# delldu/VSTNet

Measured on AMD Instinct MI355X. Metric: stylized frames/sec at 1024x1024 (1/2/4/8 GPU) + % HBM roofline, higher is better.
Workload: dtype bf16x3

## Files before the change

### include/vstnet.h

```cpp
#ifndef VSTNET_H
#define VSTNET_H

#include <stddef.h>
#include <stdint.h>

#ifdef __cplusplus
extern "C" {
#endif
#pragma GCC visibility push(default)

#define VST_OK 0
#define VST_E_ARG (-1)
#define VST_E_SHAPE (-2)
#define VST_E_MODE (-3)
#define VST_E_WORKSPACE (-4)

#define VST_PREC_BF16X3 0
#define VST_PREC_FP32 1
#define VST_PREC_F16X2 2

#define VST_PREC_F16X2H 3

#define VST_NUM_BLOCKS 32

// ... 128 lines not shown
int vst_cwct_factor_n(const double* content_stats, const double* const* style_stats_host_array, const float* alphas_host,
                      int n_styles, float alpha_c, float eps, int N, float* affine, int* info, void* workspace,
                      size_t workspace_bytes, void* stream);
int vst_cwct_prefactor_n(const double* stats, int N, float eps, double* out, int* info, void* workspace, size_t workspace_bytes,
                         void* stream);
int vst_cwct_apply_n(const float* x, float* y, int N, long L, const float* affine, const uint8_t* mask, int label, void* stream);
size_t vst_cwct_stats_n_f64_workspace_bytes(int N, long L);
int vst_cwct_stats_n_f64(const float* x, int N, long L, const uint8_t* mask, int label, double* stats, void* workspace,
                         size_t workspace_bytes, void* stream);
size_t vst_cwct_factor_n_f64_workspace_bytes(int N);
int vst_cwct_factor_n_f64(const double* content_stats, const double* const* style_stats_host_array, const float* alphas_host,
                          int n_styles, float alpha_c, float eps, int N, double* affine, int* info, void* workspace,
                          size_t workspace_bytes, void* stream);
int vst_cwct_apply_n_f64(const float* x, float* y, int N, long L, const double* affine, const uint8_t* mask, int label,
                         void* stream);

#define VST_KERNEL_ID(cin, cout, stride) (((cin) << 16) | ((cout) << 4) | (stride))
#define VST_KERNEL_ALL (-1)
#define VST_KERNEL_PACK 1
#define VST_KERNEL_UNPACK 2
#define VST_KERNEL_SPREAD 3
#define VST_KERNEL_GATHER 4
#define VST_KERNEL_CWCT_STATS 5
#define VST_KERNEL_CWCT_FACTOR 6
#define VST_KERNEL_CWCT_APPLY 7
#define VST_KERNEL_PRESPLIT 8
int vst_profile_begin(int kernel_id, int max_records);
int vst_profile_end(double* total_ms, int* launches);
int vst_profile_end_table(int* ids, double* ms, int* launches, int cap, int* n_ids);

#define VST_OPT_STAGE3_LEAN 1
#define VST_OPT_STAGE3_PINGPONG 2
#define VST_OPT_STAGE3_WIDE 3
int vst_set_option(int option, int value);
int vst_get_option(int option);

#pragma GCC visibility pop
#ifdef __cplusplus
}
#endif
#endif
```

### vstnet_amd/_lib.py

```python
from __future__ import annotations

import ctypes as C
import glob
import os
import subprocess

PKG_DIR = os.path.dirname(os.path.abspath(__file__))
REPO_DIR = os.path.dirname(PKG_DIR)
LIB_PATH = os.environ.get("VSTNET_HIP_LIB") or os.path.join(PKG_DIR, "libvstnet_hip.so")
RESOURCES_PATH = os.path.join(PKG_DIR, "libvstnet_hip.resources.txt")
SOURCES = sorted(glob.glob(os.path.join(PKG_DIR, "csrc", "*.hip")))
HEADERS = sorted(glob.glob(os.path.join(PKG_DIR, "csrc", "*.h"))) + [os.path.join(REPO_DIR, "include", "vstnet.h")]

NUM_BLOCKS = 32
PREC_BF16X3 = 0
PREC_FP32 = 1
PREC_F16X2 = 2
PREC_F16X2H = 3

EXPORTS = [
    "vst_version", "vst_error_string", "vst_conv_packed_bytes", "vst_pack_conv", "vst_pack_input",
    "vst_unpack_output", "vst_pack_input_u8", "vst_unpack_output_u8", "vst_revnet_forward_u8", "vst_revnet_inverse_u8",
    "vst_spread", "vst_gather", "vst_block_tmp_bytes", "vst_block_apply",
    "vst_pass_workspace_bytes", "vst_revnet_forward", "vst_revnet_inverse",
    "vst_cwct_stats_workspace_bytes", "vst_cwct_stats", "vst_cwct_factor", "vst_cwct_apply", "vst_cwct_apply_prec",
    "vst_cwct_prefactor", "vst_label_plan", "vst_cwct_labels_workspace_bytes", "vst_cwct_stats_labels",
    "vst_cwct_factor_labels", "vst_cwct_apply_labels", "vst_profile_begin", "vst_profile_end", "vst_profile_end_table", "vst_lab_luminance",
    "vst_revnet_encode", "vst_revnet_encode_u8", "vst_revnet_decode", "vst_revnet_decode_u8", "vst_code_to_z", "vst_z_to_code",
    "vst_cwct_stats_code_workspace_bytes", "vst_cwct_stats_code", "vst_cwct_apply_code",
    "vst_mask_to_code", "vst_cwct_stats_labels_code_workspace_bytes", "vst_cwct_stats_labels_code", "vst_cwct_apply_labels_code",
    "vst_revnet_decode_labels", "vst_revnet_decode_labels_u8", "vst_pass_sub_batch",
    "vst_normalize_block", "vst_range_flags", "vst_range_flags_async",
    "vst_cwct_stats_f64_workspace_bytes", "vst_cwct_stats_f64", "vst_cwct_factor_f64_workspace_bytes", "vst_cwct_factor_f64",
    "vst_cwct_apply_f64",
    "vst_generic_conv", "vst_generic_squeeze", "vst_generic_unsqueeze", "vst_generic_copy_channels", "vst_generic_zero",
    "vst_set_option", "vst_get_option",
    "vst_cwct_stats_n_workspace_bytes", "vst_cwct_stats_n", "vst_cwct_factor_n_workspace_bytes", "vst_cwct_factor_n",
    "vst_cwct_prefactor_n", "vst_cwct_apply_n", "vst_cwct_stats_n_f64_workspace_bytes", "vst_cwct_stats_n_f64",
    "vst_cwct_factor_n_f64_workspace_bytes", "vst_cwct_factor_n_f64", "vst_cwct_apply_n_f64",
    "vst_max_frame_pixels", "vst_cwct_stats_code_rect", "vst_cwct_stats_labels_code_rect",
]
OPT_STAGE3_LEAN = 1
OPT_STAGE3_PINGPONG = 2
OPT_STAGE3_WIDE = 3
RANGE_SATURATED = 1
RANGE_WEIGHT = 2


PRECISIONS = {"bf16x3": PREC_BF16X3, "fp32": PREC_FP32, "f16x2": PREC_F16X2, "f16x2h": PREC_F16X2H}


def default_precision() -> str:
    p = os.environ.get("VST_PRECISION", "bf16x3")
    if p not in PRECISIONS:
        raise ValueError(f"VST_PRECISION must be one of {sorted(PRECISIONS)}")
    return p


class VstError(RuntimeError):
    pass


class ConvWeights(C.Structure):
    _fields_ = [("packed", C.c_void_p), ("bias", C.c_void_p)]


class BlockWeights(C.Structure):
    _fields_ = [("conv", ConvWeights * 3)]


class NetWeights(C.Structure):
    _fields_ = [("blocks", BlockWeights * NUM_BLOCKS)]


def build(force: bool = False, verbose: bool = False) -> str:
    newest_src = max(os.path.getmtime(p) for p in SOURCES + HEADERS)
    if not force and os.path.exists(LIB_PATH) and os.path.getmtime(LIB_PATH) >= newest_src:
# ... 185 lines not shown
```

### vstnet_amd/csrc/conv.hip

```cpp
#include <mutex>
#include <stdlib.h>
#include "common.h"

#ifndef VST_ABLATE
#define VST_ABLATE 0
#endif

struct ConvArgs {
    const float* in;
    float* out;
    const unsigned char* packed;
    const float* bias;
    int Hin, Win, Hout, Wout;
    int Wq;
    size_t in_img_stride;
    size_t out_img_stride;
    float sign;
    int tiles_x, tiles_y, tiles_total;
    const unsigned char* packed1;
    const float* bias1;
    unsigned char* out_sp;
    size_t out_sp_img_bytes;
    unsigned trace_base;
};
// ... 721 lines not shown
        vst_pp_clk[2 * (i_)] = __builtin_amdgcn_s_memtime();                                                     \
        vst_pp_clk[2 * (i_) + 1] = __builtin_amdgcn_s_memrealtime();                                             \
    }
#else
#define PP_STAMP(grp_, st_, k_)
#define PP_CLK(i_)
#endif
template <int CIN, int COUT, int NW_ = 8, int MR_ = 2>
struct PipeCfg {
    static constexpr int NW = NW_, NTHR = 64 * NW, MR = MR_;
    static constexpr int NT = 64, NB = 4, TH = MR * NW, IW = 18, NPIX = (TH + 2) * IW, NSLOT = (NPIX + 15) / 16 * 16;
    static constexpr int NCHUNK = CIN / 32, NCOT = COUT / 64;
    static constexpr int A_PLANE = 4 * NSLOT * 16, A_BUF = 2 * A_PLANE;
    static constexpr int B_PLANE = 3 * 4 * 64 * 16, B_BUF = 2 * B_PLANE;
    static constexpr int LDS_BYTES = 2 * A_BUF + 2 * B_BUF;
    static constexpr int A_PART = NPIX * 4 / 3;
    static constexpr int A_ITEMS = ((A_PART / 4 + 15) / 16 * 64 + NTHR - 1) / NTHR;
    static constexpr int B_ITEMS = 2 * 768 / NTHR;
    static_assert(NPIX % 3 == 0, "three equal parts");
    static_assert(LDS_BYTES <= 160 * 1024, "LDS budget");
};

template <int NDSR, int NVM, int NDW>
__device__ __forceinline__ void wide_interleave() {
#pragma unroll
    for (int i = 0; i < 48; ++i) {
        __builtin_amdgcn_sched_group_barrier(0x008, 1, 0);
        if (i % 2 == 0 && i / 2 < NDSR) __builtin_amdgcn_sched_group_barrier(0x100, 1, 0);
        if (i % 2 == 1 && i / 2 < NVM) __builtin_amdgcn_sched_group_barrier(0x020, 1, 0);
        if (i % 2 == 1 && i / 2 < NDW) __builtin_amdgcn_sched_group_barrier(0x200, 1, 0);
    }
}

template <int CIN, int COUT, bool IN_STATE, bool OUT_STATE, int NW = 8, int MR = 2>
__global__ __launch_bounds__(64 * NW, (NW == 4 && MR == 2) ? 2 : 1) void conv_pipe_kernel(const ConvArgs a) {
    using C = PipeCfg<CIN, COUT, NW, MR>;
    constexpr bool WIDE = NW == 4 && MR == 4;
    extern __shared__ __attribute__((aligned(16))) unsigned char smem[];
    unsigned char* const Abuf = smem;
    unsigned char* const Bbuf = smem + 2 * C::A_BUF;

    const int tid = threadIdx.x, lane = tid & 63, wave = tid >> 6;
    const int lrow = lane & 15, kg = lane >> 4;
    int bx, by, b;
    if (!xcd_tile(a, bx, by, b)) return;
    VST_TRACE_BEGIN(4)
    PP_CLK(0)
    const int tx0 = bx * 16, ty0 = by * C::TH;
    const float* const in_img = a.in + (size_t)b * a.in_img_stride;
    float* const out_img = a.out + (size_t)b * a.out_img_stride;
    const PackedConvLayout PL = packed_conv_layout(COUT, CIN);
    const unsigned char* const w_plane0 = a.packed + PL.f32_bytes;

    unsigned a_src[3][C::A_ITEMS], a_dst[3][C::A_ITEMS];
#pragma unroll
    for (int part = 0; part < 3; ++part)
#pragma unroll
        for (int it = 0; it < C::A_ITEMS; ++it) {
            const int j = it * C::NTHR + tid;
            int sl = (j >> 6) * 16 + (j & 15);
            sl = sl < C::A_PART / 4 ? sl : C::A_PART / 4 - 1;
            const int cig = (j >> 4) & 3, slot = part * (C::A_PART / 4) + sl;
            const int iy = slot / C::IW, ix = slot - iy * C::IW;
            const int gy = reflect_clamp(ty0 - 1 + iy, a.Hin), gx = reflect_clamp(tx0 - 1 + ix, a.Win);
            const size_t off = IN_STATE ? zc_offset(vst_level_of_channels(CIN), gy, gx, a.Wq)
                                        : ((size_t)gy * a.Win + gx) * CIN;
            a_src[part][it] = (unsigned)(off + cig * 8);
            a_dst[part][it] = (cig * C::NSLOT + slot) * 16;
        }
    typedef f32x4 APart[C::A_ITEMS][2];
    typedef u32x4 BStage[C::B_ITEMS];
#define LOAD_A(r, chunk, part)                                                          \
    _Pragma("unroll") for (int it_ = 0; it_ < C::A_ITEMS; ++it_) {                      \
// ... 22 lines not shown
            const int k3 = r >> 8, kgi = (r >> 6) & 3, co = r & 63;
            b_off[it] = (int)(plane * PL.frag_bytes) + ((k3 * 4 + kgi) * COUT + co) * 16;
            b_dst[it] = plane * C::B_PLANE + r * 16;
        }
    }
#define LOAD_B(r, q_, dy_)                                                              \
    {                                                                                   \
        const int cot_ = (q_) / C::NCHUNK, chunk_ = (q_) - cot_ * C::NCHUNK;            \
        const unsigned char* src_ = w_plane0 + ((size_t)(chunk_ * 9 + (dy_) * 3) * 4 * COUT + cot_ * 64) * 16;   \
        _Pragma("unroll") for (int it_ = 0; it_ < C::B_ITEMS; ++it_) r[it_] = *(const u32x4*)(src_ + b_off[it_]); \
    }
#define STORE_B(buf, r)                                                                 \
    { _Pragma("unroll") for (int it_ = 0; it_ < C::B_ITEMS; ++it_) *(u32x4*)(Bbuf + (buf) * C::B_BUF + b_dst[it_]) = r[it_]; }
    struct Frags { bf16x8 wh[4], wl[4], xh[C::MR], xl[C::MR]; };
    auto read_frags = [&](Frags& f, const unsigned char* Ab, const unsigned char* Bb, int k3) {
#pragma unroll
        for (int n = 0; n < 4; ++n) {
            f.wh[n] = __builtin_bit_cast(bf16x8, *(const uint4*)(Bb + (k3 * 256 + n * 16) * 16));
            f.wl[n] = __builtin_bit_cast(bf16x8, *(const uint4*)(Bb + C::B_PLANE + (k3 * 256 + n * 16) * 16));
        }
#pragma unroll
        for (int m = 0; m < C::MR; ++m) {
            f.xh[m] = __builtin_bit_cast(bf16x8, *(const uint4*)(Ab + (m * C::IW + k3) * 16));
            f.xl[m] = __builtin_bit_cast(bf16x8, *(const uint4*)(Ab + C::A_PLANE + (m * C::IW + k3) * 16));
        }
    };

    constexpr int Q = C::NCOT * C::NCHUNK;
    static_assert(Q % 2 == 0, "stage parity is static only for an even number of (slice, chunk) pairs");
    constexpr bool ONE_SET = NW == 4 && !WIDE;
#define RS(i_) (ONE_SET ? 0 : (i_))
    BStage rb[ONE_SET ? 1 : 2];
    APart ra[ONE_SET ? 1 : 2];
    {
        BStage rb0;
        LOAD_B(rb0, 0, 0);
        APart r0, r1, r2;
        LOAD_A(r0, 0, 0); LOAD_A(r1, 0, 1); LOAD_A(r2, 0, 2);
        LOAD_B(rb[RS(1)], 0, 1);
        if (C::NCHUNK > 1) LOAD_A(ra[RS(1)], 1, 0);
        STORE_A(0, 0, r0); STORE_A(0, 1, r1); STORE_A(0, 2, r2);
        STORE_B(0, rb0);
    }
    __syncthreads();

    f32x4 acc[C::MR][4];
#pragma unroll
    for (int m = 0; m < C::MR; ++m)
#pragma unroll
        for (int n = 0; n < 4; ++n) acc[m][n] = f32x4{0.f, 0.f, 0.f, 0.f};
    const int slot_base = (wave * C::MR) * C::IW + lrow;
    const int oy0 = ty0 + wave * C::MR;
    float4 bias[4], old[C::MR][4];
#if VST_ABLATE & 8
    f32x16 abl_big[2];
#pragma unroll
    for (int i = 0; i < 16; ++i) { abl_big[0][i] = 0.f; abl_big[1][i] = 0.f; }
#endif
    const bool full_tile = ty0 + C::TH <= a.Hout && tx0 + 16 <= a.Wout;
    constexpr bool DEFER = OUT_STATE && C::NCOT > 1 && C::NCHUNK == 2 && !VST_PIPE_NO_DEFER;
    bool pending = false;
    int pend_cot = 0;
#define DEFER_UNIT(unit_)                                                                                                             \
    {                                                                                                                                 \
        const int m_ = (unit_) >> 2, n_ = (unit_) & 3;                                                                                \
        if (pending) {                                                             \
            float4* p_ = full_tile ? out_ptr<COUT, OUT_STATE, true>(a, out_img, oy0 + m_, tx0 + lrow, pend_cot * 64 + 4 * kg + n_ * 16) \
                                   : out_ptr<COUT, OUT_STATE, false>(a, out_img, oy0 + m_, tx0 + lrow, pend_cot * 64 + 4 * kg + n_ * 16); \
            if (full_tile || p_) *p_ = old[m_][n_];                                                                                   \
        }                                                                                                                             \
        if (VST_PIPE_OLD_SPREAD) {                                             \
            const float4* q_ = full_tile ? out_ptr<COUT, OUT_STATE, true>(a, out_img, oy0 + m_, tx0 + lrow, cot * 64 + 4 * kg + n_ * 16) \
                                         : out_ptr<COUT, OUT_STATE, false>(a, out_img, oy0 + m_, tx0 + lrow, cot * 64 + 4 * kg + n_ * 16); \
            old[m_][n_] = (full_tile || q_) ? *q_ : make_float4(0.f, 0.f, 0.f, 0.f);                                                  \
        }                                                                                                                             \
    }

#pragma unroll 1
    for (int q0 = 0; q0 < Q; q0 += 2) {
#pragma unroll
      for (int qq = 0; qq < 2; ++qq) {
        const int q = q0 + qq;
        const int cot = q / C::NCHUNK, chunk = q - cot * C::NCHUNK;
        const bool last_chunk = chunk == C::NCHUNK - 1;
#pragma unroll
        for (int dy = 0; dy < 3; ++dy) {
            const int s = q * 3 + dy;
            const int cur = (qq * 3 + dy) & 1;
            if constexpr (WIDE) {
                constexpr bool A_ALWAYS = C::NCOT == 1;
                const int q2 = dy == 0 ? q : q + 1, dy2 = (dy + 2) % 3;
                const int qn = dy == 2 ? q + 1 : q, dyn = (dy + 1) % 3;
                if (DEFER ? (dy == 2 && last_chunk) : (dy == 0 && chunk == 0)) load_bias<COUT, 4>(a, cot * 64 + 4 * kg, bias);
                if (!A_ALWAYS && q < C::NCHUNK - 1) STORE_A((chunk + 1) & 1, dy, ra[cur ^ 1]);
                if (!A_ALWAYS && qn < C::NCHUNK - 1) LOAD_A(ra[cur], qn + 1, dyn);
                if (OUT_STATE && !(DEFER && VST_PIPE_OLD_SPREAD) && dy == 2 && last_chunk) {
                    if (full_tile) load_old<COUT, C::MR, 4, true>(a, out_img, oy0, tx0 + lrow, cot * 64 + 4 * kg, old);
                    else load_old<COUT, C::MR, 4, false>(a, out_img, oy0, tx0 + lrow, cot * 64 + 4 * kg, old);
                }
                const unsigned char* Ab = Abuf + (chunk & 1) * C::A_BUF + (kg * C::NSLOT + slot_base + dy * C::IW) * 16;
                const unsigned char* Bb = Bbuf + (s & 1) * C::B_BUF + (kg * 64 + lrow) * 16;
                Frags fr[2];
#pragma unroll
                for (int k3 = 0; k3 < 3; ++k3) {
                    if constexpr (DEFER) {
                        if (qq == 0 && dy * 3 + k3 < C::MR * 2) { DEFER_UNIT(2 * (dy * 3 + k3)); DEFER_UNIT(2 * (dy * 3 + k3) + 1); }
                    }
                    if (k3 == 0) read_frags(fr[0], Ab, Bb, 0);
                    __builtin_amdgcn_sched_barrier(0);
                    if (k3 == 0) {
                        LOAD_B(rb[cur], q2 < Q ? q2 : Q - 1, dy2);
                        if (A_ALWAYS) LOAD_A(ra[cur], qn + 1 < C::NCHUNK ? qn + 1 : C::NCHUNK - 1, dyn);
                    }
                    if (k3 < 2) read_frags(fr[(k3 + 1) & 1], Ab, Bb, k3 + 1);
                    if (k3 == 2) {
                        STORE_B((s + 1) & 1, rb[cur ^ 1]);
                        if (A_ALWAYS) STORE_A((chunk + 1) & 1, dy, ra[cur ^ 1]);
                    }
                    const Frags& f = fr[k3 & 1];
#pragma unroll
                    for (int m = 0; m < C::MR; ++m)
#pragma unroll
                        for (int n = 0; n < 4; ++n) { MFMA3(acc[m][n], f.wh[n], f.wl[n], f.xh[m], f.xl[m]); }
                    constexpr int NSTG = A_ALWAYS ? C::B_ITEMS + 2 * C::A_ITEMS : C::B_ITEMS;
                    if (k3 == 0) wide_interleave<16, NSTG, 0>();
                    else if (k3 == 1) wide_interleave<16, 0, 0>();
                    else wide_interleave<0, 0, NSTG>();
                    __builtin_amdgcn_sched_barrier(0);
// ... 67 lines not shown
            } else
            if (dy == 2 && last_chunk && (!(VST_ABLATE & 4) || cot == C::NCOT - 1)) {
                if (full_tile) store_tile<COUT, OUT_STATE, C::MR, 4, true>(a, out_img, oy0, tx0 + lrow, cot * 64 + 4 * kg, acc, bias, old);
                else store_tile<COUT, OUT_STATE, C::MR, 4, false>(a, out_img, oy0, tx0 + lrow, cot * 64 + 4 * kg, acc, bias, old);
#pragma unroll
                for (int m = 0; m < C::MR; ++m)
#pragma unroll
                    for (int n = 0; n < 4; ++n) acc[m][n] = f32x4{0.f, 0.f, 0.f, 0.f};
            }
            if (DEFER && qq == 0 && dy == 2) pending = false;
            if ((VST_ABLATE & 4) && dy == 2 && last_chunk && cot != C::NCOT - 1) {
#pragma unroll
                for (int m = 0; m < C::MR; ++m)
#pragma unroll
                    for (int n = 0; n < 4; ++n) asm volatile("" : "+v"(acc[m][n]));
            }
            if (!(VST_ABLATE & 16)) __syncthreads();
        }
      }
    }
#undef LOAD_A
#undef STORE_A
#undef LOAD_B
#undef STORE_B
#undef F4_
#undef RS
#undef DEFER_UNIT
#if VST_ABLATE & 8
    asm volatile("" :: "v"(abl_big[0]), "v"(abl_big[1]));
#endif
    PP_CLK(1)
    VST_TRACE_END_(4, CIN, COUT)
}

#ifndef VST_WITH_PINGPONG
#define VST_WITH_PINGPONG 0
#endif
#if VST_WITH_PINGPONG
template <int CIN, int COUT, bool IN_STATE, bool OUT_STATE>
__global__ __launch_bounds__(512) void conv_pp_kernel(const ConvArgs a) {
    using C = PipeCfg<CIN, COUT, 8>;
    constexpr int SY = 256;
    constexpr int A_ITEMS_Y = ((C::A_PART / 4 + 15) / 16 * 64 + SY - 1) / SY;
    constexpr int B_ITEMS_Y = 2 * 768 / SY;
    extern __shared__ __attribute__((aligned(16))) unsigned char smem[];
    unsigned char* const Abuf = smem;
    unsigned char* const Bbuf = smem + 2 * C::A_BUF;
    float* const bias_lds = (float*)(smem + C::LDS_BYTES);

    const int tid = threadIdx.x, lane = tid & 63, wave = __builtin_amdgcn_readfirstlane(tid >> 6);
    const int lrow = lane & 15, kg = lane >> 4;
    const bool grpY = wave >= 4;
    int bx, by, b;
    if (!xcd_tile(a, bx, by, b)) return;
    VST_TRACE_BEGIN(4)
    PP_CLK(0)
    const int tx0 = bx * 16, ty0 = by * C::TH;
    const float* const in_img = a.in + (size_t)b * a.in_img_stride;
    float* const out_img = a.out + (size_t)b * a.out_img_stride;
    const PackedConvLayout PL = packed_conv_layout(COUT, CIN);
    const unsigned char* const w_plane0 = a.packed + PL.f32_bytes;
    constexpr int Q = C::NCOT * C::NCHUNK, S = 3 * Q;
    constexpr bool A_IN_LOOP = C::NCHUNK > 2;

#define PP_A_ADDR(j_, part_, src_, dst_)                                                                         \
    {                                                                                                            \
// ... 298 lines not shown
static int g_prof_id[VST_PROFILE_MAX_RECORDS];
static hipEvent_t g_prof_ev[2 * VST_PROFILE_MAX_RECORDS];
static bool g_prof_ev_created = false;

int vst_prof_open(int kernel_id, hipStream_t st) {
    const int sel = g_prof_kernel.load(std::memory_order_relaxed);
    if (sel != kernel_id && sel != VST_KERNEL_ALL) return -1;
    std::lock_guard<std::mutex> lk(g_prof_mu);
    if ((g_prof_kernel.load() != kernel_id && g_prof_kernel.load() != VST_KERNEL_ALL) || g_prof_count >= g_prof_cap) return -1;
    const int rec = g_prof_count++;
    g_prof_id[rec] = kernel_id;
    (void)hipEventRecord(g_prof_ev[2 * rec], st);
    return rec;
}

void vst_prof_close(int rec, hipStream_t st) {
    std::lock_guard<std::mutex> lk(g_prof_mu);
    if (rec < g_prof_count) (void)hipEventRecord(g_prof_ev[2 * rec + 1], st);
}

#ifndef VST_LEAN_DEFAULT
#define VST_LEAN_DEFAULT 0
#endif
static std::atomic<int> g_opt_lean{[] { const char* e = getenv("VST_LEAN"); return e && (e[0] == '0' || e[0] == '1') ? e[0] - '0' : VST_LEAN_DEFAULT; }()};
static bool vst_lean_stage3() { return g_opt_lean.load(std::memory_order_relaxed) != 0; }
#ifndef VST_WIDE_DEFAULT
#define VST_WIDE_DEFAULT 1
#endif
static std::atomic<int> g_opt_wide{[] { const char* e = getenv("VST_WIDE"); return e && (e[0] == '0' || e[0] == '1') ? e[0] - '0' : VST_WIDE_DEFAULT; }()};
#ifndef VST_PINGPONG_DEFAULT
#define VST_PINGPONG_DEFAULT 0
#endif
static std::atomic<int> g_opt_pp{[] { const char* e = getenv("VST_PINGPONG"); return e && (e[0] == '0' || e[0] == '1') ? e[0] - '0' : VST_PINGPONG_DEFAULT; }()};

template <int CIN, int COUT, int STRIDE, bool IN_STATE, bool OUT_STATE>
static int launch_conv(const ConvArgs& a, int B, int precision, hipStream_t st, bool out_h16 = false) {
    if (precision == VST_PREC_FP32) {
        const size_t total = (size_t)B * a.Hout * a.Wout * COUT;
        size_t blocks = (total + 255) / 256;
        if (blocks > 65536) blocks = 65536;
        conv_fp32_kernel<IN_STATE, OUT_STATE><<<dim3((unsigned)blocks), 256, 0, st>>>(a, CIN, COUT, STRIDE, B);
        VST_RETURN_IF_LAUNCH_FAILED();
        return VST_OK;
    }
    if (precision != VST_PREC_BF16X3 && !vst_is_f16(precision)) return VST_E_MODE;
    vst_prof_scope prof(VST_KERNEL_ID(CIN, COUT, STRIDE), st);
    if constexpr (CIN >= 64 && COUT >= 64 && STRIDE == 1) {
        ConvArgs t = a;
        t.tiles_x = (a.Wout + 15) / 16;
        if (vst_lean_stage3()) {
            using C = PipeCfg<CIN, COUT, 4>;
            auto kern = conv_pipe_kernel<CIN, COUT, IN_STATE, OUT_STATE, 4>;
            static std::atomic<unsigned> attr_done{0};
            if (int rc_ = vst_ensure_dynamic_lds((const void*)kern, (int)(C::LDS_BYTES), &attr_done)) return rc_;
            t.tiles_y = (a.Hout + C::TH - 1) / C::TH; t.tiles_total = t.tiles_x * t.tiles_y * B;
            VST_TRACE_RESERVE(t, (t.tiles_total + 7) / 8 * 8)
            kern<<<dim3((t.tiles_total + 7) / 8 * 8), C::NTHR, C::LDS_BYTES, st>>>(t);
        } else if (g_opt_wide.load(std::memory_order_relaxed)) {
            using C = PipeCfg<CIN, COUT, 4, 4>;
            auto kern = conv_pipe_kernel<CIN, COUT, IN_STATE, OUT_STATE, 4, 4>;
            static std::atomic<unsigned> attr_done{0};
            if (int rc_ = vst_ensure_dynamic_lds((const void*)kern, (int)(C::LDS_BYTES), &attr_done)) return rc_;
            t.tiles_y = (a.Hout + C::TH - 1) / C::TH; t.tiles_total = t.tiles_x * t.tiles_y * B;
            VST_TRACE_RESERVE(t, (t.tiles_total + 7) / 8 * 8)
            kern<<<dim3((t.tiles_total + 7) / 8 * 8), C::NTHR, C::LDS_BYTES, st>>>(t);
#if VST_WITH_PINGPONG
// ... 65 lines not shown
template <int MID, int CH>
static int launch_pair(const ConvArgs& a, int B, int precision, hipStream_t st) {
    constexpr int T2 = 2;
    const bool t2 = T2 == 2 && vst_is_f16(precision);
    if (precision == VST_PREC_F16X2H) {
        using P = PairCfg<MID, CH, 2, 4, true>;
        vst_prof_scope prof(VST_KERNEL_ID(MID, CH, 1), st);
        auto kern = conv_pair_kernel<MID, CH, 2, 4, true>;
        static std::atomic<unsigned> attr_h16{0};
        if (int rc_ = vst_ensure_dynamic_lds((const void*)kern, P::LDS_BYTES, &attr_h16)) return rc_;
        ConvArgs t = a;
        t.tiles_x = (a.Wout + 15) / 16; t.tiles_y = (a.Hout + 15) / 16; t.tiles_total = t.tiles_x * t.tiles_y * B;
        VST_TRACE_RESERVE(t, (t.tiles_total + 7) / 8 * 8)
        kern<<<dim3((t.tiles_total + 7) / 8 * 8), 256, P::LDS_BYTES, st>>>(t);
        VST_RETURN_IF_LAUNCH_FAILED();
        return VST_OK;
    }
    vst_prof_scope prof(VST_KERNEL_ID(MID, CH, 1), st);
    constexpr int MRT = (MID == 16 && VST_PAIR_MR2) ? 2 : 4;
    constexpr int MRT3 = (MID == 16 && VST_PAIR_MR2_T3) ? 2 : 4;
    auto kern = t2 ? conv_pair_kernel<MID, CH, T2, MRT> : conv_pair_kernel<MID, CH, 3, MRT3>;
    const int lds = t2 ? PairCfg<MID, CH, T2, MRT>::LDS_BYTES : PairCfg<MID, CH, 3, MRT3>::LDS_BYTES;
    const int th = t2 ? 4 * MRT : 4 * MRT3;
    static std::atomic<unsigned> attr_done[2];
    if (int rc_ = vst_ensure_dynamic_lds((const void*)kern, lds, &attr_done[t2 ? 1 : 0])) return rc_;
    ConvArgs t = a;
    t.tiles_x = (a.Wout + 15) / 16; t.tiles_y = (a.Hout + th - 1) / th; t.tiles_total = t.tiles_x * t.tiles_y * B;
    VST_TRACE_RESERVE(t, (t.tiles_total + 7) / 8 * 8)
    kern<<<dim3((t.tiles_total + 7) / 8 * 8), 256, lds, st>>>(t);
    VST_RETURN_IF_LAUNCH_FAILED();
    return VST_OK;
}

template <int CH, int STRIDE>
static int run_block(const vst_block_weights* w, int direction, int precision, float* dst, const float* src,
                     float* tmp, int B, int H, int W, hipStream_t st) {
    constexpr int LV = CH == 16 ? 0 : (CH == 64 ? 1 : 2);
    constexpr int MID = CH / 4;
    constexpr int IN_CH = STRIDE == 1 ? CH : CH / 4;
    const int Ho = H >> LV, Wo = W >> LV;
    const size_t state_img = (size_t)H * W * 16;
    const size_t mid_img = (size_t)Ho * Wo * MID;
    float* h1 = tmp;
    float* h2 = tmp + (size_t)B * mid_img;
    ConvArgs a{};
    a.Wq = W >> 2;
    a.in = src; a.out = h1; a.packed = (const unsigned char*)w->conv[0].packed; a.bias = w->conv[0].bias;
    a.Hin = Ho * STRIDE; a.Win = Wo * STRIDE; a.Hout = Ho; a.Wout = Wo;
    a.in_img_stride = state_img; a.out_img_stride = mid_img; a.sign = 0.f;
    if constexpr (CH == 256 && STRIDE == 2) {
        if (vst_is_f16(precision)) {
            const size_t mid_bytes = (size_t)Ho * Wo * 64 * 4, state_bytes = (size_t)Ho * Wo * 256 * 4;
            unsigned char* const h1p = (unsigned char*)tmp;
            unsigned char* const h2p = h1p + (size_t)B * mid_bytes;
            unsigned char* const planes_a = h2p + (size_t)B * mid_bytes;
            (void)state_bytes;
            a.out_sp = h1p; a.out_sp_img_bytes = mid_bytes;
            int rc2 = launch_conv_s2_planes(a, B, st);
            if (rc2) return rc2;
            const int h2_single = precision == VST_PREC_F16X2H;
            rc2 = vst3_conv_mid(&w->conv[1], h1p, h2p, h2_single, B, H, W, st);
            if (rc2) return rc2;
            return vst3_conv_out(&w->conv[2], h2p, h2_single, dst, direction > 0 ? planes_a : nullptr, direction > 0 ? 1.f : -1.f,
                                 B, H, W, st);
        }
    }
    const bool h16 = CH <= 64 && VST_PAIR && precision == VST_PREC_F16X2H;
    int rc = launch_conv<IN_CH, MID, STRIDE, true, false>(a, B, precision, st, h16);
    if (rc) return rc;
    if constexpr (CH <= 64 && VST_PAIR) {
        if (precision != VST_PREC_FP32) {
            a.in = h1; a.out = dst; a.Hin = Ho; a.Win = Wo; a.in_img_stride = mid_img; a.out_img_stride = state_img;
            a.packed = (const unsigned char*)w->conv[2].packed; a.bias = w->conv[2].bias;
            a.packed1 = (const unsigned char*)w->conv[1].packed; a.bias1 = w->conv[1].bias;
            a.sign = direction > 0 ? 1.f : -1.f;
            return launch_pair<MID, CH>(a, B, precision, st);
        }
    }
    a.in = h1; a.out = h2; a.packed = (const unsigned char*)w->conv[1].packed; a.bias = w->conv[1].bias;
    a.Hin = Ho; a.Win = Wo; a.in_img_stride = mid_img;
    rc = launch_conv<MID, MID, 1, false, false>(a, B, precision, st);
    if (rc) return rc;
    a.in = h2; a.out = dst; a.packed = (const unsigned char*)w->conv[2].packed; a.bias = w->conv[2].bias;
    a.out_img_stride = state_img; a.sign = direction > 0 ? 1.f : -1.f;
    return launch_conv<MID, CH, 1, false, true>(a, B, precision, st);
}

static const int kBlockChannel[VST_NUM_BLOCKS] = {16, 16, 16, 16, 16, 16, 16, 16, 16, 16, 64, 64, 64, 64, 64, 64,
                                                  64, 64, 64, 64, 256, 256, 256, 256, 256, 256, 256, 256, 256, 256,
                                                  256, 256};
static const int kBlockStride[VST_NUM_BLOCKS] = {1, 1, 1, 1, 1, 1, 1, 1, 1, 1, 2, 1, 1, 1, 1, 1,
                                                 1, 1, 1, 1, 2, 1, 1, 1, 1, 1, 1, 1, 1, 1, 1, 1};

VST_DEFINE_TU_RANGE(vst_range_tu_conv)

extern "C" {

int vst_set_option(int option, int value) {
    if (option == VST_OPT_STAGE3_LEAN) g_opt_lean.store(value != 0, std::memory_order_relaxed);
    else if (option == VST_OPT_STAGE3_WIDE) g_opt_wide.store(value != 0, std::memory_order_relaxed);
    else if (option == VST_OPT_STAGE3_PINGPONG && VST_WITH_PINGPONG) g_opt_pp.store(value != 0, std::memory_order_relaxed);
    else return VST_E_ARG;
    return VST_OK;
}

int vst_get_option(int option) {
    if (option == VST_OPT_STAGE3_LEAN) return g_opt_lean.load(std::memory_order_relaxed);
    if (option == VST_OPT_STAGE3_WIDE) return g_opt_wide.load(std::memory_order_relaxed);
    if (option == VST_OPT_STAGE3_PINGPONG && VST_WITH_PINGPONG) return g_opt_pp.load(std::memory_order_relaxed);
    return VST_E_ARG;
}

int vst_range_flags(unsigned* flags_host, int reset) {
    if (!flags_host) return VST_E_ARG;
    hipError_t e = hipDeviceSynchronize();
    if (e != hipSuccess) return (int)e;
    unsigned v = 0;
    if (int rc = vst_range_tu_conv(&v, reset)) return rc;
    if (int rc = vst_range_tu_conv3(&v, reset)) return rc;
    if (int rc = vst_range_tu_layout(&v, reset)) return rc;
    if (int rc = vst_range_tu_cwct(&v, reset)) return rc;
    *flags_host = v;
    return VST_OK;
}

int vst_range_flags_async(unsigned* flags4_dev, void* stream) {
    if (!flags4_dev) return VST_E_ARG;
    hipStream_t st = (hipStream_t)stream;
    if (int rc = vst_range_tu_conv_async(flags4_dev + 0, st)) return rc;
    if (int rc = vst_range_tu_conv3_async(flags4_dev + 1, st)) return rc;
    if (int rc = vst_range_tu_layout_async(flags4_dev + 2, st)) return rc;
    return vst_range_tu_cwct_async(flags4_dev + 3, st);
}

int vst_profile_begin(int kernel_id, int max_records) {
    if ((kernel_id <= 0 && kernel_id != VST_KERNEL_ALL) || max_records <= 0) return VST_E_ARG;
    if (max_records > VST_PROFILE_MAX_RECORDS) max_records = VST_PROFILE_MAX_RECORDS;
    std::lock_guard<std::mutex> lk(g_prof_mu);
    if (!g_prof_ev_created) {
        for (int i = 0; i < 2 * VST_PROFILE_MAX_RECORDS; ++i) {
            hipError_t e = hipEventCreate(&g_prof_ev[i]);
            if (e != hipSuccess) return (int)e;
// ... 335 lines not shown
```

### vstnet_amd/csrc/layout.hip

```cpp
#include "common.h"

__global__ __launch_bounds__(256) void pack_input_kernel(const float* __restrict__ x, float* __restrict__ s1,
                                                         int C, int H, int W, const float* __restrict__ addk) {
    const int xg = blockIdx.x * 64 + (threadIdx.x & 63);
    const int yg = blockIdx.y * 4 + (threadIdx.x >> 6);
    const int b = blockIdx.z;
    if (xg >= W || yg >= H) return;
    const size_t plane = (size_t)H * W;
    const float* src = x + (size_t)b * C * plane + (size_t)yg * W + xg;
    float v[16];
#pragma unroll
    for (int c = 0; c < 16; ++c) v[c] = (c < C ? src[c * plane] : 0.f) + (addk ? addk[c] : 0.f);
    float* dst = s1 + (size_t)b * plane * 16 + zc_offset(0, yg, xg, W >> 2);
#pragma unroll
    for (int c = 0; c < 16; c += 4) *(float4*)(dst + c) = make_float4(v[c], v[c + 1], v[c + 2], v[c + 3]);
}

__global__ __launch_bounds__(256) void unpack_output_kernel(const float* __restrict__ s1, float* __restrict__ x,
                                                            int C, int H, int W) {
    const int xg = blockIdx.x * 64 + (threadIdx.x & 63);
    const int yg = blockIdx.y * 4 + (threadIdx.x >> 6);
    const int b = blockIdx.z;
    if (xg >= W || yg >= H) return;
    const size_t plane = (size_t)H * W;
// ... 199 lines not shown
}

__global__ __launch_bounds__(256) void normalize_block_kernel(float* __restrict__ w1, float* __restrict__ b1, float* __restrict__ w4,
                                                              float* __restrict__ b4, float* __restrict__ w7, int cin1, int mid,
                                                              int cout, float* __restrict__ scales) {
    __shared__ float sc[64];
    const int tid = threadIdx.x, lane = tid & 63, wave = tid >> 6;
    auto row_scales = [&](const float* w, int K) {
        for (int r = wave; r < mid; r += 4) {
            float acc = 0.f;
            for (int k = lane; k < K; k += 64) { const float v = w[(size_t)r * K + k]; acc += v * v; }
#pragma unroll
            for (int o = 32; o >= 1; o >>= 1) acc += __shfl_xor(acc, o, 64);
            if (lane == 0) sc[r] = pow2_scale_of_norm(acc);
        }
        __syncthreads();
    };
    const int K1 = cin1 * 9, K4 = mid * 9;
    row_scales(w1, K1);
    for (int i = tid; i < mid * K1; i += 256) w1[i] *= sc[i / K1];
    for (int i = tid; i < mid; i += 256) { b1[i] *= sc[i]; if (scales) scales[i] = sc[i]; }
    for (int i = tid; i < mid * K4; i += 256) w4[i] /= sc[(i / 9) % mid];
    __syncthreads();
    row_scales(w4, K4);
    for (int i = tid; i < mid * K4; i += 256) w4[i] *= sc[i / K4];
    for (int i = tid; i < mid; i += 256) { b4[i] *= sc[i]; if (scales) scales[mid + i] = sc[i]; }
    for (int i = tid; i < cout * K4; i += 256) w7[i] /= sc[(i / 9) % mid];
}

VST_DEFINE_TU_RANGE(vst_range_tu_layout)

extern "C" {

int vst_version(void) { return 104; }
int64_t vst_max_frame_pixels(void) { return VST_MAX_FRAME_PIXELS; }

int vst_normalize_block(float* w1, float* b1, float* w4, float* b4, float* w7, int c_in1, int c_mid, int c_out, float* scales,
                        void* stream) {
    if (!w1 || !b1 || !w4 || !b4 || !w7) return VST_E_ARG;
    if (c_in1 <= 0 || c_mid <= 0 || c_mid > 64 || c_out <= 0) return VST_E_SHAPE;
    normalize_block_kernel<<<dim3(1), 256, 0, (hipStream_t)stream>>>(w1, b1, w4, b4, w7, c_in1, c_mid, c_out, scales);
    VST_RETURN_IF_LAUNCH_FAILED();
    return VST_OK;
}

const char* vst_error_string(int code) {
    switch (code) {
        case VST_OK: return "ok";
        case VST_E_ARG: return "invalid argument (null pointer or non-positive size)";
        case VST_E_SHAPE: return "unsupported shape (H, W must be multiples of 4 and >= 8, H * W <= VST_MAX_FRAME_PIXELS; channels in the documented sets)";
        case VST_E_MODE: return "unknown mode (precision / sp_steps / direction)";
        case VST_E_WORKSPACE: return "workspace too small or null";
        default: return code > 0 ? hipGetErrorString((hipError_t)code) : "unknown vstnet error";
    }
}

size_t vst_conv_packed_bytes(int cout, int cin) {
    const PackedConvLayout L = packed_conv_layout(cout, cin);
    return L.f16_offset + L.frag_bytes;
}

int vst_pack_conv(const float* w, int cout, int cin, void* packed, void* stream) {
    if (!w || !packed || cout <= 0) return VST_E_ARG;
    if (!(cin == 4 || cin == 16 || (cin >= 32 && cin % 32 == 0))) return VST_E_SHAPE;
    const PackedConvLayout L = packed_conv_layout(cout, cin);
    size_t n = (size_t)9 * cin * cout;
    const size_t n_frag = (size_t)L.ksteps * 4 * L.coutp * 8;
// ... 98 lines not shown
```

Measured before the change: 221.2.

## Fuse conv.4 into conv.7 for 256-channel stage-3 blocks via LDS halo tile

For 256-channel blocks in bf16x3 with the wide path, the middle 64->64 conv is now computed inside the 64->256 conv kernel. Each tile loads a 20x20 halo of h1 into LDS, computes the 18x18 h2 region (interior plus ring) with MFMA, applies bias, ReLU and reflect padding, and writes h2 into LDS where the next conv reads it. This removes the h2 round-trip through HBM and one launch, at the cost of recomputing halo pixels, higher LDS use and register pressure. It is on by default and can be turned off through an option or environment variable.

```diff
diff --git a/include/vstnet.h b/include/vstnet.h
--- a/include/vstnet.h
+++ b/include/vstnet.h
@@ -184,6 +184,7 @@
 #define VST_OPT_STAGE3_LEAN 1
 #define VST_OPT_STAGE3_PINGPONG 2
 #define VST_OPT_STAGE3_WIDE 3
+#define VST_OPT_STAGE3_PAIR 4
 int vst_set_option(int option, int value);
 int vst_get_option(int option);
 
diff --git a/vstnet_amd/_lib.py b/vstnet_amd/_lib.py
--- a/vstnet_amd/_lib.py
+++ b/vstnet_amd/_lib.py
@@ -43,6 +43,7 @@
 OPT_STAGE3_LEAN = 1
 OPT_STAGE3_PINGPONG = 2
 OPT_STAGE3_WIDE = 3
+OPT_STAGE3_PAIR = 4
 RANGE_SATURATED = 1
 RANGE_WEIGHT = 2
 
diff --git a/vstnet_amd/csrc/conv.hip b/vstnet_amd/csrc/conv.hip
--- a/vstnet_amd/csrc/conv.hip
+++ b/vstnet_amd/csrc/conv.hip
@@ -777,13 +777,67 @@
     }
 }
 
-template <int CIN, int COUT, bool IN_STATE, bool OUT_STATE, int NW = 8, int MR = 2>
+struct S3PairCfg {
+    static constexpr int R1 = 20, N1SLOT = R1 * R1;
+    static constexpr int A1_PLANE = 4 * N1SLOT * 16, A1_BUF = 2 * A1_PLANE;
+    static constexpr int H1_ITEMS = (4 * N1SLOT + 255) / 256;
+    static constexpr int NRING = 2 * 18 + 2 * 16;
+    static constexpr int B_OFF = 2 * A1_BUF;
+    static constexpr int LDS_BYTES = B_OFF + 2 * PipeCfg<64, 256, 4, 4>::B_BUF;
+    static_assert(2 * PipeCfg<64, 256, 4, 4>::A_BUF <= B_OFF, "the h2 images fit over the h1 images");
+    static_assert(LDS_BYTES <= 160 * 1024, "LDS budget");
+};
+
+__device__ __forceinline__ void s3_ring_pos(int p, int& ry, int& rx) {
+    if (p < 36) {
+        ry = p < 18 ? 0 : 17;
+        rx = p < 18 ? p : p - 18;
+    } else {
+        ry = (p < 52 ? p - 36 : p - 52) + 1;
+        rx = p < 52 ? 0 : 17;
+    }
+}
+
+__device__ __forceinline__ void s3_put_h2(unsigned char* smem, const f32x4& acc, const float4& bias, int n, int kg, int ry, int rx,
+                                          bool ok, bool ring_in, int ty0, int tx0, int H, int W) {
+    using C7 = PipeCfg<64, 256, 4, 4>;
+    float4 r = make_float4(acc[0] + bias.x, acc[1] + bias.y, acc[2] + bias.z, acc[3] + bias.w);
+    r.x = r.x > 0.f ? r.x : 0.f; r.y = r.y > 0.f ? r.y : 0.f;
+    r.z = r.z > 0.f ? r.z : 0.f; r.w = r.w > 0.f ? r.w : 0.f;
+    uint2 h, l;
+    split4(r, h, l);
+    unsigned char* const base = smem + (n >> 1) * C7::A_BUF + ((n & 1) * 2 + (kg >> 1)) * C7::NSLOT * 16 + (kg & 1) * 8;
+#define S3_PUT(slot_)                                                                              \
+    {                                                                                              \
+        *(uint2*)(base + (slot_) * 16) = h;                                                        \
+        *(uint2*)(base + C7::A_PLANE + (slot_) * 16) = l;                                          \
+    }
+    if (ring_in) {
+        if (ok) S3_PUT(ry * C7::IW + rx);
+    } else {
+        const int gy = ty0 - 1 + ry, gx = tx0 - 1 + rx;
+        if (ok && gy >= 0 && gy < H && gx >= 0 && gx < W) {
+            const int my = gy == 1 ? -2 : (gy == H - 2 ? 2 : 0), mx = gx == 1 ? -2 : (gx == W - 2 ? 2 : 0);
+            int sy = ry + my, sx = rx + mx;
+            sy = (sy < 0 || sy >= 18) ? ry : sy;
+            sx = (sx < 0 || sx >= 18) ? rx : sx;
+            S3_PUT(ry * C7::IW + rx);
+            S3_PUT(sy * C7::IW + rx);
+            S3_PUT(ry * C7::IW + sx);
+            S3_PUT(sy * C7::IW + sx);
+        }
+    }
+#undef S3_PUT
+}
+
+template <int CIN, int COUT, bool IN_STATE, bool OUT_STATE, int NW = 8, int MR = 2, bool S3PAIR = false>
 __global__ __launch_bounds__(64 * NW, (NW == 4 && MR == 2) ? 2 : 1) void conv_pipe_kernel(const ConvArgs a) {
     using C = PipeCfg<CIN, COUT, NW, MR>;
     constexpr bool WIDE = NW == 4 && MR == 4;
+    static_assert(!S3PAIR || (WIDE && CIN == 64 && COUT == 256 && !IN_STATE && OUT_STATE), "the fused form: conv.7 of the 256-channel blocks");
     extern __shared__ __attribute__((aligned(16))) unsigned char smem[];
     unsigned char* const Abuf = smem;
-    unsigned char* const Bbuf = smem + 2 * C::A_BUF;
+    unsigned char* const Bbuf = smem + (S3PAIR ? S3PairCfg::B_OFF : 2 * C::A_BUF);
 
     const int tid = threadIdx.x, lane = tid & 63, wave = tid >> 6;
     const int lrow = lane & 15, kg = lane >> 4;
@@ -872,7 +926,128 @@
 #define RS(i_) (ONE_SET ? 0 : (i_))
     BStage rb[ONE_SET ? 1 : 2];
     APart ra[ONE_SET ? 1 : 2];
-    {
+    if constexpr (S3PAIR) {
+        using S = S3PairCfg;
+        const PackedConvLayout PL4 = packed_conv_layout(64, 64);
+        const unsigned char* const w4_plane0 = a.packed1 + PL4.f32_bytes;
+        int b4_off[C::B_ITEMS];
+#pragma unroll
+        for (int it = 0; it < C::B_ITEMS; ++it) {
+            const int plane = it / 3, k3 = it % 3, kgi = tid >> 6, co = tid & 63;
+            b4_off[it] = ((kgi * 64 + co) * 16) + (int)(plane * PL4.frag_bytes) + k3 * 4 * 64 * 16;
+        }
+#define LOAD_B4(r, s_)                                                                                              \
+        {                                                                                                           \
+            const unsigned char* src_ = w4_plane0 + (size_t)(((s_) / 3) * 9 + ((s_) % 3) * 3) * 4 * 64 * 16;       \
+            _Pragma("unroll") for (int it_ = 0; it_ < C::B_ITEMS; ++it_) r[it_] = *(const u32x4*)(src_ + b4_off[it_]); \
+        }
+        {
+            f32x4 hr[2][S::H1_ITEMS][2];
+#define H1_ITEM(c_, it_)                                                                                            \
+            int j_ = (it_) * 256 + tid;                                                                             \
+            j_ = j_ < 4 * S::N1SLOT ? j_ : 4 * S::N1SLOT - 1;                                                       \
+            const int sl_ = (j_ >> 6) * 16 + (j_ & 15), cig_ = (j_ >> 4) & 3;
+#pragma unroll
+            for (int c = 0; c < 2; ++c)
+#pragma unroll
+                for (int it = 0; it < S::H1_ITEMS; ++it) {
+                    H1_ITEM(c, it)
+                    const int iy = sl_ / S::R1, ix = sl_ - iy * S::R1;
+                    const int gy = reflect_clamp(ty0 - 2 + iy, a.Hin), gx = reflect_clamp(tx0 - 2 + ix, a.Win);
+                    const float* p = in_img + ((size_t)gy * a.Win + gx) * 64 + c * 32 + cig_ * 8;
+                    hr[c][it][0] = *(const f32x4*)p;
+                    hr[c][it][1] = *(const f32x4*)(p + 4);
+                }
+            BStage rb0;
+            LOAD_B4(rb0, 0);
+            LOAD_B4(rb[1], 1);
+#pragma unroll
+            for (int c = 0; c < 2; ++c)
+#pragma unroll
+                for (int it = 0; it < S::H1_ITEMS; ++it) {
+                    H1_ITEM(c, it)
+                    unsigned char* const d = smem + c * S::A1_BUF + (cig_ * S::N1SLOT + sl_) * 16;
+                    uint4 h, l;
+                    split8(F4_(hr[c][it][0]), F4_(hr[c][it][1]), h, l);
+                    *(uint4*)d = h;
+                    *(uint4*)(d + S::A1_PLANE) = l;
+                }
+#undef H1_ITEM
+            STORE_B(0, rb0);
+        }
+        __syncthreads();
+
+        f32x4 acc4[4][4], accr[4], accx;
+#pragma unroll
+        for (int m = 0; m < 4; ++m)
+#pragma unroll
+            for (int n = 0; n < 4; ++n) acc4[m][n] = f32x4{0.f, 0.f, 0.f, 0.f};
+#pragma unroll
+        for (int n = 0; n < 4; ++n) accr[n] = f32x4{0.f, 0.f, 0.f, 0.f};
+        accx = f32x4{0.f, 0.f, 0.f, 0.f};
+        int pry, prx, pxy, pxx;
+        s3_ring_pos(wave * 16 + lrow, pry, prx);
+        const bool x_ok = lrow < S::NRING - 64;
+        s3_ring_pos(x_ok ? 64 + lrow : S::NRING - 1, pxy, pxx);
+        const unsigned char* const Xt = smem + (kg * S::N1SLOT + (wave * 4 + 1) * S::R1 + lrow + 1) * 16;
+        const unsigned char* const Xr = smem + (kg * S::N1SLOT + pry * S::R1 + prx) * 16;
+        const unsigned char* const Xx = smem + (kg * S::N1SLOT + pxy * S::R1 + pxx) * 16;
+        const unsigned char* const Wf = Bbuf + (kg * 64 + lrow) * 16;
+#pragma unroll 1
+        for (int s0 = 0; s0 < 6; s0 += 2) {
+#pragma unroll
+          for (int par = 0; par < 2; ++par) {
+            const int s = s0 + par, c = s / 3, dy = s - 3 * c;
+            if (s + 2 < 6) { LOAD_B4(rb[par], s + 2); }
+            else LOAD_B(rb[par], 0, s - 4);
+            const int xo = c * S::A1_BUF + dy * S::R1 * 16;
+            const unsigned char* const Bb = Wf + par * C::B_BUF;
+#pragma unroll
+            for (int k3 = 0; k3 < 3; ++k3) {
+                bf16x8 wh[4], wl[4], xh[4], xl[4], rh, rl, qh, ql, vh, vl;
+#pragma unroll
+                for (int n = 0; n < 4; ++n) {
+                    wh[n] = __builtin_bit_cast(bf16x8, *(const uint4*)(Bb + (k3 * 256 + n * 16) * 16));
+                    wl[n] = __builtin_bit_cast(bf16x8, *(const uint4*)(Bb + C::B_PLANE + (k3 * 256 + n * 16) * 16));
+                }
+#pragma unroll
+                for (int m = 0; m < 4; ++m) {
+                    xh[m] = __builtin_bit_cast(bf16x8, *(const uint4*)(Xt + xo + (m * S::R1 + k3) * 16));
+                    xl[m] = __builtin_bit_cast(bf16x8, *(const uint4*)(Xt + xo + S::A1_PLANE + (m * S::R1 + k3) * 16));
+                }
+                rh = __builtin_bit_cast(bf16x8, *(const uint4*)(Xr + xo + k3 * 16));
+                rl = __builtin_bit_cast(bf16x8, *(const uint4*)(Xr + xo + S::A1_PLANE + k3 * 16));
+                qh = __builtin_bit_cast(bf16x8, *(const uint4*)(Xx + xo + k3 * 16));
+                ql = __builtin_bit_cast(bf16x8, *(const uint4*)(Xx + xo + S::A1_PLANE + k3 * 16));
+                vh = __builtin_bit_cast(bf16x8, *(const uint4*)(Bb + (k3 * 256 + wave * 16) * 16));
+                vl = __builtin_bit_cast(bf16x8, *(const uint4*)(Bb + C::B_PLANE + (k3 * 256 + wave * 16) * 16));
+#pragma unroll
+                for (int m = 0; m < 4; ++m)
+#pragma unroll
+                    for (int n = 0; n < 4; ++n) { MFMA3(acc4[m][n], wh[n], wl[n], xh[m], xl[m]); }
+#pragma unroll
+                for (int n = 0; n < 4; ++n) { MFMA3(accr[n], wh[n], wl[n], rh, rl); }
+                MFMA3(accx, vh, vl, qh, ql);
+            }
+            STORE_B(par ^ 1, rb[par ^ 1]);
+            __syncthreads();
+          }
+        }
+#undef LOAD_B4
+        float4 b4[4];
+#pragma unroll
+        for (int n = 0; n < 4; ++n) b4[n] = *(const float4*)(a.bias1 + n * 16 + 4 * kg);
+        const int H = a.Hout, W = a.Wout;
+        const bool ring_in = ty0 >= 1 && tx0 >= 1 && ty0 + 17 <= H && tx0 + 17 <= W;
+#pragma unroll
+        for (int m = 0; m < 4; ++m)
+#pragma unroll
+            for (int n = 0; n < 4; ++n) s3_put_h2(smem, acc4[m][n], b4[n], n, kg, wave * 4 + m + 1, lrow + 1, true, ring_in, ty0, tx0, H, W);
+#pragma unroll
+        for (int n = 0; n < 4; ++n) s3_put_h2(smem, accr[n], b4[n], n, kg, pry, prx, true, ring_in, ty0, tx0, H, W);
+        const float4 bx4 = *(const float4*)(a.bias1 + wave * 16 + 4 * kg);
+        s3_put_h2(smem, accx, bx4, wave, kg, pxy, pxx, x_ok, ring_in, ty0, tx0, H, W);
+    } else {
         BStage rb0;
         LOAD_B(rb0, 0, 0);
         APart r0, r1, r2;
@@ -932,8 +1107,8 @@
                 const int q2 = dy == 0 ? q : q + 1, dy2 = (dy + 2) % 3;
                 const int qn = dy == 2 ? q + 1 : q, dyn = (dy + 1) % 3;
                 if (DEFER ? (dy == 2 && last_chunk) : (dy == 0 && chunk == 0)) load_bias<COUT, 4>(a, cot * 64 + 4 * kg, bias);
-                if (!A_ALWAYS && q < C::NCHUNK - 1) STORE_A((chunk + 1) & 1, dy, ra[cur ^ 1]);
-                if (!A_ALWAYS && qn < C::NCHUNK - 1) LOAD_A(ra[cur], qn + 1, dyn);
+                if (!A_ALWAYS && !S3PAIR && q < C::NCHUNK - 1) STORE_A((chunk + 1) & 1, dy, ra[cur ^ 1]);
+                if (!A_ALWAYS && !S3PAIR && qn < C::NCHUNK - 1) LOAD_A(ra[cur], qn + 1, dyn);
                 if (OUT_STATE && !(DEFER && VST_PIPE_OLD_SPREAD) && dy == 2 && last_chunk) {
                     if (full_tile) load_old<COUT, C::MR, 4, true>(a, out_img, oy0, tx0 + lrow, cot * 64 + 4 * kg, old);
                     else load_old<COUT, C::MR, 4, false>(a, out_img, oy0, tx0 + lrow, cot * 64 + 4 * kg, old);
@@ -1067,6 +1242,8 @@
     PP_CLK(1)
     VST_TRACE_END_(4, CIN, COUT)
 }
+
+
 
 #ifndef VST_WITH_PINGPONG
 #define VST_WITH_PINGPONG 0
@@ -1431,6 +1608,10 @@
 #define VST_PINGPONG_DEFAULT 0
 #endif
 static std::atomic<int> g_opt_pp{[] { const char* e = getenv("VST_PINGPONG"); return e && (e[0] == '0' || e[0] == '1') ? e[0] - '0' : VST_PINGPONG_DEFAULT; }()};
+#ifndef VST_S3PAIR_DEFAULT
+#define VST_S3PAIR_DEFAULT 1
+#endif
+static std::atomic<int> g_opt_s3pair{[] { const char* e = getenv("VST_S3PAIR"); return e && (e[0] == '0' || e[0] == '1') ? e[0] - '0' : VST_S3PAIR_DEFAULT; }()};
 
 template <int CIN, int COUT, int STRIDE, bool IN_STATE, bool OUT_STATE>
 static int launch_conv(const ConvArgs& a, int B, int precision, hipStream_t st, bool out_h16 = false) {
@@ -1562,6 +1743,19 @@
     return VST_OK;
 }
 
+static int launch_s3pair(const ConvArgs& a, int B, hipStream_t st) {
+    vst_prof_scope prof(VST_KERNEL_ID(64, 256, 1), st);
+    constexpr int lds = S3PairCfg::LDS_BYTES;
+    static std::atomic<unsigned> attr_done{0};
+    if (int rc_ = vst_ensure_dynamic_lds((const void*)conv_pipe_kernel<64, 256, false, true, 4, 4, true>, lds, &attr_done)) return rc_;
+    ConvArgs t = a;
+    t.tiles_x = (a.Wout + 15) / 16; t.tiles_y = (a.Hout + 15) / 16; t.tiles_total = t.tiles_x * t.tiles_y * B;
+    VST_TRACE_RESERVE(t, (t.tiles_total + 7) / 8 * 8)
+    conv_pipe_kernel<64, 256, false, true, 4, 4, true><<<dim3((t.tiles_total + 7) / 8 * 8), 256, lds, st>>>(t);
+    VST_RETURN_IF_LAUNCH_FAILED();
+    return VST_OK;
+}
+
 template <int CH, int STRIDE>
 static int run_block(const vst_block_weights* w, int direction, int precision, float* dst, const float* src,
                      float* tmp, int B, int H, int W, hipStream_t st) {
@@ -1607,6 +1801,16 @@
             return launch_pair<MID, CH>(a, B, precision, st);
         }
     }
+    if constexpr (CH == 256) {
+        if (precision == VST_PREC_BF16X3 && !vst_lean_stage3() && g_opt_wide.load(std::memory_order_relaxed) &&
+            g_opt_s3pair.load(std::memory_order_relaxed)) {
+            a.in = h1; a.out = dst; a.Hin = Ho; a.Win = Wo; a.in_img_stride = mid_img; a.out_img_stride = state_img;
+            a.packed = (const unsigned char*)w->conv[2].packed; a.bias = w->conv[2].bias;
+            a.packed1 = (const unsigned char*)w->conv[1].packed; a.bias1 = w->conv[1].bias;
+            a.sign = direction > 0 ? 1.f : -1.f;
+            return launch_s3pair(a, B, st);
+        }
+    }
     a.in = h1; a.out = h2; a.packed = (const unsigned char*)w->conv[1].packed; a.bias = w->conv[1].bias;
     a.Hin = Ho; a.Win = Wo; a.in_img_stride = mid_img;
     rc = launch_conv<MID, MID, 1, false, false>(a, B, precision, st);
@@ -1630,6 +1834,7 @@
     if (option == VST_OPT_STAGE3_LEAN) g_opt_lean.store(value != 0, std::memory_order_relaxed);
     else if (option == VST_OPT_STAGE3_WIDE) g_opt_wide.store(value != 0, std::memory_order_relaxed);
     else if (option == VST_OPT_STAGE3_PINGPONG && VST_WITH_PINGPONG) g_opt_pp.store(value != 0, std::memory_order_relaxed);
+    else if (option == VST_OPT_STAGE3_PAIR) g_opt_s3pair.store(value != 0, std::memory_order_relaxed);
     else return VST_E_ARG;
     return VST_OK;
 }
@@ -1638,6 +1843,7 @@
     if (option == VST_OPT_STAGE3_LEAN) return g_opt_lean.load(std::memory_order_relaxed);
     if (option == VST_OPT_STAGE3_WIDE) return g_opt_wide.load(std::memory_order_relaxed);
     if (option == VST_OPT_STAGE3_PINGPONG && VST_WITH_PINGPONG) return g_opt_pp.load(std::memory_order_relaxed);
+    if (option == VST_OPT_STAGE3_PAIR) return g_opt_s3pair.load(std::memory_order_relaxed);
     return VST_E_ARG;
 }
 
diff --git a/vstnet_amd/csrc/layout.hip b/vstnet_amd/csrc/layout.hip
--- a/vstnet_amd/csrc/layout.hip
+++ b/vstnet_amd/csrc/layout.hip
@@ -255,7 +255,7 @@
 
 extern "C" {
 
-int vst_version(void) { return 104; }
+int vst_version(void) { return 105; }
 int64_t vst_max_frame_pixels(void) { return VST_MAX_FRAME_PIXELS; }
 
 int vst_normalize_block(float* w1, float* b1, float* w4, float* b4, float* w7, int c_in1, int c_mid, int c_out, float* scales,
```

Measured after the change: 220.6, median of 2. No clear change (-0.3%).
